# SarodYatawatta/federated-pytorch-test

Hardware: NVIDIA H100
Metric: train_images_per_sec (higher is better)
Workload: dtype tf32

## Files before the change

### federated_pytorch_test_b200/_ext.py

```python
from __future__ import annotations

import importlib.util
import os
import sys
import threading
from typing import Dict, List

_HERE = os.path.dirname(os.path.abspath(__file__))
_CSRC = os.path.join(_HERE, "csrc")
_BUILD = os.path.join(_HERE, "_build")

CUDA_ARCH_FLAGS = ["-gencode", "arch=compute_90a,code=sm_90a"]
NVCC_FLAGS = ["-O3", "-lineinfo", "--use_fast_math", "-std=c++17", "--expt-relaxed-constexpr",
              "-Xptxas", "-v"] + CUDA_ARCH_FLAGS
CXX_FLAGS = ["-O3", "-std=c++17", "-fPIC"]

_SPECS: Dict[str, Dict] = {
    "fedb200_runtime": {"sources": ["batch_loader.cpp"], "cuda": False},
    "fedb200_cuda": {
        "sources": ["bindings.cpp", "flat_kernels.cu", "elementwise_kernels.cu", "norm_kernels.cu", "loss_kernels.cu",
                    "comm_kernels.cu", "gemm_wgmma.cu", "aux_kernels.cu"],
        "cuda": True,
    },
}

_loaded: Dict[str, object] = {}
_lock = threading.Lock()


def _sources(name: str) -> List[str]:
    return [os.path.join(_CSRC, s) for s in _SPECS[name]["sources"] if os.path.exists(os.path.join(_CSRC, s))]


def _so_path(name: str) -> str:
    return os.path.join(_BUILD, name, name + ".so")


def _stale(name: str) -> bool:
    so = _so_path(name)
    if not os.path.exists(so):
        return True
    t = os.path.getmtime(so)
    deps = _sources(name) + [os.path.join(_CSRC, f) for f in os.listdir(_CSRC) if f.endswith((".cuh", ".h", ".hpp"))]
    return any(os.path.getmtime(s) > t for s in deps)
# ... 59 lines not shown
```

### federated_pytorch_test_b200/csrc/bindings.cpp

```cpp
#include <ATen/cuda/CUDAContext.h>
#include <c10/cuda/CUDAGuard.h>
#include <torch/extension.h>

#include <cstdlib>

#include "fedb200.h"

namespace fb = fedb200;
using torch::Tensor;

static cudaStream_t cur_stream() { return at::cuda::getCurrentCUDAStream().stream(); }
static const float* fptr(const Tensor& t) { return t.data_ptr<float>(); }
static float* fptr_mut(Tensor& t) { return t.data_ptr<float>(); }
static const float* opt_ptr(const c10::optional<Tensor>& t) { return (t.has_value() && t->defined()) ? t->data_ptr<float>() : nullptr; }

#define CHECK_F32_CUDA(x) TORCH_CHECK((x).is_cuda() && (x).scalar_type() == torch::kFloat32, #x " must be a CUDA float32 tensor")
#define CHECK_CONTIG(x) TORCH_CHECK((x).is_contiguous(), #x " must be contiguous")

void adam_prox(Tensor x, Tensor g, Tensor m, Tensor v, Tensor step, double lr, double b1, double b2, double eps,
               c10::optional<Tensor> z, c10::optional<Tensor> y, double rho, double l1, double l2,
               c10::optional<Tensor> rho_dev, c10::optional<Tensor> lr_dev, double weight_decay,
               c10::optional<Tensor> norm_dev, double clip) {
  CHECK_F32_CUDA(x); CHECK_CONTIG(x); CHECK_CONTIG(g); CHECK_CONTIG(m); CHECK_CONTIG(v);
  c10::cuda::CUDAGuard guard(x.device());
// ... 183 lines not shown
  fb::col_stats(fptr(y), fptr_mut(stats), (int)(y.numel() / C), C, cur_stream());
}
std::vector<Tensor> bn_elu_fwd(Tensor y, c10::optional<Tensor> stats, Tensor gamma, Tensor beta, c10::optional<Tensor> residual,
                               c10::optional<Tensor> running_mean, c10::optional<Tensor> running_var, double eps,
                               double momentum, bool act, bool self_clean, bool use_running) {
  CHECK_F32_CUDA(y); CHECK_CONTIG(y);
  c10::cuda::CUDAGuard guard(y.device());
  const int C = (int)y.size(-1);
  const int M = (int)(y.numel() / C);
  auto out = torch::empty_like(y);
  float* rm = (running_mean.has_value() && running_mean->defined()) ? running_mean->data_ptr<float>() : nullptr;
  float* rv = (running_var.has_value() && running_var->defined()) ? running_var->data_ptr<float>() : nullptr;
  if (use_running) {
    TORCH_CHECK(rm != nullptr && rv != nullptr, "bn_elu_fwd: use_running needs running_mean and running_var");
    fb::bn_elu_fwd(fptr(y), nullptr, fptr(gamma), fptr(beta), opt_ptr(residual), fptr_mut(out), rm, rv, nullptr, nullptr, M, C,
                   (float)eps, 0.f, act ? 1 : 0, 0, cur_stream(), 1);
    return {out, Tensor(), Tensor()};
  }
  TORCH_CHECK(stats.has_value() && stats->defined(), "bn_elu_fwd: stats required");
  auto sm = torch::empty({C}, y.options()), si = torch::empty({C}, y.options());
  TORCH_CHECK(stats->numel() >= 2 * C + (self_clean ? 1 : 0), "stats buffer too small");
  fb::bn_elu_fwd(fptr(y), stats->data_ptr<float>(), fptr(gamma), fptr(beta), opt_ptr(residual), fptr_mut(out), rm, rv, fptr_mut(sm),
                 fptr_mut(si), M, C, (float)eps, (float)momentum, act ? 1 : 0, self_clean ? 1 : 0, cur_stream());
  return {out, sm, si};
}
std::vector<Tensor> bn_elu_bwd(Tensor dout, c10::optional<Tensor> out, Tensor y, Tensor mean, Tensor invstd, Tensor gamma,
                               c10::optional<Tensor> beta, c10::optional<Tensor> dgamma, c10::optional<Tensor> dbeta,
                               bool want_dres, bool act, c10::optional<Tensor> sums_buf) {
  CHECK_F32_CUDA(dout); CHECK_CONTIG(dout); CHECK_CONTIG(y);
  c10::cuda::CUDAGuard guard(y.device());
  const int C = (int)y.size(-1);
  const int M = (int)(y.numel() / C);
  const float* outp = nullptr;
  if (out.has_value() && out->defined()) { CHECK_CONTIG((*out)); outp = out->data_ptr<float>(); }
  const float* betap = opt_ptr(beta);
  const bool persistent = sums_buf.has_value() && sums_buf->defined();
  if (persistent) TORCH_CHECK(sums_buf->numel() == 2 * C + 1 && sums_buf->is_contiguous(), "bn_elu_bwd: sums buffer must be [2C + 1]");
  auto sums = persistent ? *sums_buf : torch::empty({2 * C + 1}, y.options());
  auto dy = torch::empty_like(y);
  Tensor dres;
  if (want_dres) dres = torch::empty_like(y);
  float* dg = (dgamma.has_value() && dgamma->defined()) ? dgamma->data_ptr<float>() : nullptr;
  float* db = (dbeta.has_value() && dbeta->defined()) ? dbeta->data_ptr<float>() : nullptr;
  fb::bn_elu_bwd_reduce(fptr(dout), outp, fptr(y), fptr(mean), fptr(invstd), fptr(gamma), betap, fptr_mut(sums), M, C,
                        act ? 1 : 0, persistent ? 1 : 0, cur_stream());
  fb::bn_elu_bwd_apply(fptr(dout), outp, fptr(y), fptr(mean), fptr(invstd), fptr(gamma), betap, fptr_mut(sums), fptr_mut(dy),
// ... 851 lines not shown
  m.def("scaffold_corr_blocks", &scaffold_corr_blocks);
  m.def("scaffold_corr", &scaffold_corr);
  m.def("bump_step", &bump_step);
  m.def("l1_l2", &l1_l2);
  m.def("make_pair", &make_pair);
  m.def("welford", &welford);
  m.def("penalty_value", &penalty_value);
  m.def("penalty_grad", &penalty_grad);
  m.def("multi_dot", &multi_dot);
  m.def("lbfgs_two_loop", &lbfgs_two_loop);
  m.def("normalize_u8", &normalize_u8);
  m.def("augment_normalize_u8", &augment_normalize_u8, py::arg("u8"), py::arg("rows"), py::arg("key"), py::arg("counter"),
        py::arg("mean"), py::arg("std"), py::arg("to_nchw"));
  m.def("mix_normalize_u8", &mix_normalize_u8, py::arg("u8"), py::arg("rows"), py::arg("augment"), py::arg("key"),
        py::arg("counter"), py::arg("mean"), py::arg("std"), py::arg("to_nchw"), py::arg("cutmix"), py::arg("lam_f"),
        py::arg("mlam_f"), py::arg("y0"), py::arg("y1"), py::arg("x0"), py::arg("x1"), py::arg("lam_eff"));
  m.def("col_stats", &col_stats);
  m.def("head_fwd", &head_fwd);
  m.def("head_bwd", &head_bwd);
  m.def("bn_elu_fwd", &bn_elu_fwd, py::arg("y"), py::arg("stats"), py::arg("gamma"), py::arg("beta"), py::arg("residual"),
        py::arg("running_mean"), py::arg("running_var"), py::arg("eps"), py::arg("momentum"), py::arg("act"),
        py::arg("self_clean"), py::arg("use_running") = false);
  m.def("bn_elu_bwd", &bn_elu_bwd);
  m.def("gn_elu_fwd", &gn_elu_fwd, py::arg("y"), py::arg("gamma"), py::arg("beta"), py::arg("residual"), py::arg("groups"),
        py::arg("eps"), py::arg("act"));
  m.def("gn_elu_bwd", &gn_elu_bwd, py::arg("dout"), py::arg("out"), py::arg("y"), py::arg("mean"), py::arg("rstd"),
        py::arg("gamma"), py::arg("beta"), py::arg("groups"), py::arg("want_dres"), py::arg("act"), py::arg("want_affine"));
  m.def("avgpool_nhwc", &avgpool_nhwc);
  m.def("avgpool_nhwc_bwd", &avgpool_nhwc_bwd);
  m.def("weight_flip", &weight_flip);
  m.def("convT_pack", &convT_pack);
  m.def("linear_tf32", &linear_tf32);
  m.def("conv_supported", &conv_supported);
  m.def("conv_orientation", &conv_orientation);
  m.def("conv_window_reuse", &conv_window_reuse, py::arg("H_out"), py::arg("W_out"), py::arg("C_in"), py::arg("C_out"), py::arg("kh"),
        py::arg("stride") = 1, py::arg("dil") = 1);
  m.def("conv2d_nhwc", &conv2d_nhwc, py::arg("x"), py::arg("w"), py::arg("stats"), py::arg("stride"), py::arg("pad"), py::arg("dil"),
        py::arg("orient") = -1);
  m.def("conv2d_nhwc_sized", &conv2d_nhwc_sized);
  m.def("conv2d_nhwc_bias_act", &conv2d_nhwc_bias_act);
  m.def("conv2d_nhwc_bn_eval", &conv2d_nhwc_bn_eval);
  m.def("conv2d_nhwc_shuffle", &conv2d_nhwc_shuffle);
  m.def("conv_shuffle_supported", &conv_shuffle_supported);
  m.def("conv2d_nhwc_multidil", &conv2d_nhwc_multidil);
  m.def("conv_multidil_supported", &conv_multidil_supported);
  m.def("conv_wgrad", &conv_wgrad);
// ... 37 lines not shown
```

### federated_pytorch_test_b200/csrc/fedb200.h

```cpp
#pragma once
#include <cuda_runtime.h>
#include <stdint.h>

namespace fedb200 {

void count_launch(int n = 1);
long long launch_count();

bool pdl_enabled();
#ifdef __CUDACC__
__device__ __forceinline__ void pdl_wait() { asm volatile("griddepcontrol.wait;" ::: "memory"); }
__device__ __forceinline__ void pdl_launch_dependents() { asm volatile("griddepcontrol.launch_dependents;" ::: "memory"); }
__device__ __forceinline__ void pdl_prologue() {
  pdl_launch_dependents();
  pdl_wait();
}
template <typename... KArgs, typename... Args>
inline cudaError_t launch_pdl(void (*kernel)(KArgs...), dim3 grid, dim3 block, size_t smem, cudaStream_t stream,
                              Args&&... args) {
  cudaLaunchConfig_t cfg{};
  cfg.gridDim = grid;
  cfg.blockDim = block;
  cfg.dynamicSmemBytes = smem;
  cfg.stream = stream;
// ... 14 lines not shown
int pick_conv_orientation(int NB, int H_out, int W_out, int C_out, int stride);
bool conv_window_reuse(int H_out, int W_out, int C_in, int C_out, int kh, int stride, int dil);
void conv2d_nhwc_tf32(const float* x, const float* w, float* y, float* stats, int NB, int H, int W, int C_in, int C_out,
                      int kh, int kw, int stride, int pad, int dil, int H_out, int W_out, cudaStream_t stream,
                      int orient = CONV_ORIENT_AUTO);
void conv2d_nhwc_bias_act_tf32(const float* x, const float* w, const float* bias, int act, float* y, int NB, int H, int W,
                               int C_in, int C_out, int kh, int kw, int stride, int pad, int dil, int H_out, int W_out,
                               cudaStream_t stream);
void conv2d_nhwc_bn_eval_tf32(const float* x, const float* w, const float* gamma, const float* beta, const float* mean,
                              const float* var, float eps, const float* residual, int act, float* y, int NB, int H, int W,
                              int C_in, int C_out, int kh, int kw, int stride, int pad, int dil, int H_out, int W_out,
                              cudaStream_t stream);

bool conv_shuffle_supported(int H_out, int W_out, int C_in, int Ci_out);
void conv2d_nhwc_shuffle_tf32(const float* x, const float* w, float* out, int NB, int H, int W, int C_in, int C4, int kh, int kw,
                              int pad, int H_out, int W_out, cudaStream_t stream);
bool conv_multidil_supported(int H_out, int W_out, int C_in, int stride, int branches);
void conv2d_nhwc_multidil_tf32(const float* x, const float* w, const float* bias, int act, float* y, int NB, int H, int W, int C_in,
                               int C_out, int branches, int kh, int kw, int stride, const int* dils, const int* pads, int H_out,
                               int W_out, cudaStream_t stream);
bool conv_wgrad_supported(int C_x, int C_out, int stride, int W_out, int H_out);
void conv_wgrad_tf32(const float* x, const float* dy, float* dw, int NB, int H, int W, int C_x, int C_w, int C_out, int kh,
                     int kw, int stride, int pad, int dil, int H_out, int W_out, cudaStream_t stream);


void adam_prox(float* x, const float* g, float* m, float* v, const int* step_dev, int n, float lr, float b1, float b2,
               float eps, const float* z, const float* y, float rho, float l1, float l2, cudaStream_t s,
               const float* rho_dev = nullptr, const float* lr_dev = nullptr, float weight_decay = 0.f,
               const float* norm_dev = nullptr, float clip = 0.f);
void sgd_prox(float* x, const float* g, float* buf, int n, float lr, float momentum, bool nesterov, float weight_decay,
              const float* z, const float* y, float rho, float l1, float l2, cudaStream_t s, const float* rho_dev,
              const float* lr_dev = nullptr, const float* norm_dev = nullptr, float clip = 0.f);
constexpr int kGradNormHeader = 4;
int grad_norm_blocks(int n);
void grad_norm(const float* g, int n, float* ws, unsigned int* ticket, float clip, cudaStream_t s);
void bump_step(int* step_dev, cudaStream_t s);
void l1_l2(const float* g, int n, float* out2, cudaStream_t s);
void make_pair(const float* g, const float* gprev, const float* d, float t, float trust, float* y, float* sv, int n,
               float* out3, cudaStream_t s);
void welford(const float* g, float* mean, float* m2, int n, float inv_n, float* out1, cudaStream_t s);
void penalty_value(const float* x, const float* z, const float* y, float rho, float l1, float l2, int n, float* out1,
                   cudaStream_t s);
void penalty_grad(float* g, const float* x, const float* z, const float* y, float rho, float l1, float l2, int n,
                  cudaStream_t s);
void multi_dot(const float* const* a, const float* const* b, int npairs, int n, float* out, cudaStream_t s);
constexpr int kTwoLoopMaxHist = 32;
// ... 241 lines not shown
```

### federated_pytorch_test_b200/csrc/gemm_wgmma.cu

```cuda
#include "fedb200.h"
#include "igemm_wgmma.cuh"
#include "wgrad_wgmma.cuh"

#include <algorithm>
#include <cstdlib>
#include <mutex>
#include <stdexcept>
#include <string>

namespace fedb200 {

typedef CUresult (*EncodeTiledFn)(CUtensorMap*, CUtensorMapDataType, cuuint32_t, void*, const cuuint64_t*,
                                  const cuuint64_t*, const cuuint32_t*, const cuuint32_t*, CUtensorMapInterleave,
                                  CUtensorMapSwizzle, CUtensorMapL2promotion, CUtensorMapFloatOOBfill);

static EncodeTiledFn encode_fn() {
  static EncodeTiledFn fn = nullptr;
  static std::once_flag once;
  std::call_once(once, [] {
    void* p = nullptr;
    cudaDriverEntryPointQueryResult q;
    cudaError_t e = cudaGetDriverEntryPoint("cuTensorMapEncodeTiled", &p, cudaEnableDefault, &q);
    if (e != cudaSuccess || q != cudaDriverEntryPointSuccess || p == nullptr)
      throw std::runtime_error("fedb200: cuTensorMapEncodeTiled unavailable (no CUDA driver?)");
// ... 402 lines not shown
    p.cw = cw;
    p.num_k_blocks = (kh_all * kw + IG_BLOCK_K / cw - 1) / (IG_BLOCK_K / cw);
  }
  p.taps_w = kw; p.b_cols_per_tap = C_in; p.is_conv = 1;
  p.HW_out = H_out * W_out; p.W_out = W_out;
  p.stride = stride; p.pad = 0; p.dil = 1;
  p.out = y; p.ldo = C_out; p.bias = bias; p.act = act; p.stats = nullptr;
  p.k_splits = 1; p.kb_per_split = p.num_k_blocks;
  p.ms_kh = kh;
  for (int b = 0; b < branches; ++b) {
    if (dils[b] < 1 || dils[b] > 255 || pads[b] < 0 || pads[b] > 255) throw std::runtime_error("fedb200: multi-dilation: dilation / padding out of range");
    p.ms_dil |= (unsigned long long)(dils[b]) << (8 * b);
    p.ms_pad |= (unsigned long long)(pads[b]) << (8 * b);
  }
  dispatch(bn, ta, tb, p, stream);
}

bool conv_wgrad_supported(int C_x, int C_out, int stride, int W_out, int H_out) {
  if ((C_x & 3) || (C_out & 3)) return false;
  if (stride < 1 || stride > 8) return false;
  return W_out > 0 && H_out > 0;
}

template <int BN>
static void launch_wgrad(const float* x, const float* dy, const WgradParams& p, int grid, cudaStream_t stream) {
  constexpr int smem = 2 * (WG_A_BYTES + BN * WG_BK * 4);
  auto kernel = wgrad_wgmma_kernel<BN>;
  static bool configured = false;
  if (!configured) {
    cudaError_t e = cudaFuncSetAttribute(kernel, cudaFuncAttributeMaxDynamicSharedMemorySize, smem);
    if (e != cudaSuccess) throw std::runtime_error(std::string("fedb200: cudaFuncSetAttribute(wgrad): ") + cudaGetErrorString(e));
    configured = true;
  }
  cudaError_t e = launch_pdl(kernel, dim3(grid), dim3(WG_THREADS), size_t(smem), stream, x, dy, p);
  if (e != cudaSuccess) throw std::runtime_error(std::string("fedb200: wgrad launch: ") + cudaGetErrorString(e));
  count_launch();
}

void conv_wgrad_tf32(const float* x, const float* dy, float* dw, int NB, int H, int W, int C_x, int C_w, int C_out, int kh,
                     int kw, int stride, int pad, int dil, int H_out, int W_out, cudaStream_t stream) {
  if (!conv_wgrad_supported(C_x, C_out, stride, W_out, H_out))
    throw std::runtime_error("fedb200: wgrad geometry not supported by the wgmma path");
  WgradParams p{};
  p.H = H; p.W = W; p.Cx = C_x; p.Cw = C_w; p.Co = C_out;
  p.kw = kw; p.stride = stride; p.pad = pad; p.dil = dil; p.H_out = H_out; p.W_out = W_out;
  p.J = kh * kw * C_w;
  p.P = NB * H_out * W_out;
  p.dw = dw;
  const int bn = C_out <= 32 ? 32 : (C_out <= 64 ? 64 : 128);
  p.j_tiles = (p.J + WG_BM - 1) / WG_BM;
  p.co_tiles = (C_out + bn - 1) / bn;
  const int kb_total = (p.P + WG_BK - 1) / WG_BK;
  const int base = p.j_tiles * p.co_tiles;
  int splits = std::max(1, 2 * num_sms() / base);
  splits = std::min(splits, std::max(1, kb_total / 8));
  splits = std::max(1, std::min(splits, kb_total));
  p.kb_per_split = (kb_total + splits - 1) / splits;
  splits = (kb_total + p.kb_per_split - 1) / p.kb_per_split;
  const int grid = base * splits;
  switch (bn) {
    case 32: launch_wgrad<32>(x, dy, p, grid, stream); break;
    case 64: launch_wgrad<64>(x, dy, p, grid, stream); break;
    default: launch_wgrad<128>(x, dy, p, grid, stream); break;
  }
}

}
```

### federated_pytorch_test_b200/csrc/wgrad_wgmma.cuh

```cuda
#pragma once
#include "sm90.cuh"

namespace fedb200 {

constexpr int WG_THREADS = 256;
constexpr int WG_BM = 128;
constexpr int WG_BK = 32;
constexpr int WG_A_BYTES = WG_BM * WG_BK * 4;

struct WgradParams {
  int H, W, Cx, Cw, Co, kw, stride, pad, dil, H_out, W_out;
  int J;
  int P;
  int kb_per_split;
  int j_tiles, co_tiles;
  float* dw;
};

__device__ __forceinline__ uint32_t wg_core_offset(int row, int k) {
  return uint32_t((row >> 3) * 1024 + (k >> 2) * 128 + (row & 7) * 16 + (k & 3) * 4);
}
__device__ __forceinline__ float to_tf32(float v) {
  uint32_t r;
  asm("cvt.rna.tf32.f32 %0, %1;" : "=r"(r) : "f"(v));
  return __uint_as_float(r);
}

template <int BN>
__global__ void __launch_bounds__(WG_THREADS, 1)
wgrad_wgmma_kernel(const float* __restrict__ x, const float* __restrict__ dy, const WgradParams p) {
  constexpr int B_BYTES = BN * WG_BK * 4;
  constexpr int BUF_BYTES = WG_A_BYTES + B_BYTES;
  constexpr int A_PER = WG_BM * WG_BK / WG_THREADS;
  constexpr int B_GROUPS = WG_THREADS / BN;
  constexpr int B_PER = WG_BK / B_GROUPS;
  constexpr int NACC = BN / 2;
  extern __shared__ __align__(1024) uint8_t smem[];

  const int tid = threadIdx.x;
  const int g = tid >> 7, warp = (tid >> 5) & 3, lane = tid & 31;
  int unit = blockIdx.x;
  const int jt = unit % p.j_tiles;
  unit /= p.j_tiles;
  const int ct = unit % p.co_tiles;
  const int split = unit / p.co_tiles;
  const int j0 = jt * WG_BM, co0 = ct * BN;
  const int kb_begin = split * p.kb_per_split;
  const int kb_total = (p.P + WG_BK - 1) / WG_BK;
  const int nkb = min(p.kb_per_split, kb_total - kb_begin);
  const int HWo = p.H_out * p.W_out;

  const int a_row = tid & (WG_BM - 1), a_pg = tid >> 7;
  const int j = j0 + a_row;
// ... 82 lines not shown
```

### federated_pytorch_test_b200/ops/cuda_ops.py

```python
from __future__ import annotations

from typing import List, Optional, Sequence, Tuple

import torch
import torch.nn as nn
import torch.nn.functional as F

from .. import _ext
from . import conv_math

_EXT = None


def ext():
    global _EXT
    if _EXT is None:
        _EXT = _ext.load("fedb200_cuda", required=True)
    return _EXT


def launch_count() -> int:
    return int(ext().launch_count())


# ... 330 lines not shown
    return bool(ext().conv_wgrad_supported(xn.shape[3], dy.shape[3], stride, dy.shape[2], dy.shape[1]))


def conv_wgrad(xn: torch.Tensor, dy: torch.Tensor, kh: int, kw: int, cw: int, stride: int, pad: int, dil: int,
               weight: Optional[torch.Tensor] = None) -> Optional[torch.Tensor]:
    Co = dy.shape[3]
    dyc = dy if dy.is_contiguous() else dy.contiguous()
    buf = _grad_buffer_krsc(weight, (Co, kh, kw, cw))
    if buf is not None:
        ext().conv_wgrad(xn, dyc, buf, stride, pad, dil)
        return None
    dwk = torch.zeros(Co, kh, kw, cw, dtype=torch.float32, device=xn.device)
    ext().conv_wgrad(xn, dyc, dwk, stride, pad, dil)
    return dwk.permute(0, 3, 1, 2)


class _ConvBnAct(torch.autograd.Function):

    @staticmethod
    def forward(ctx, x, weight, gamma, beta, residual, running_mean, running_var, stride, pad, eps, momentum, act):
        e = ext()
        xn = _nhwc(x)
        wk = _krsc(weight)
        if xn.shape[3] == 3:
            xn = F.pad(xn, (0, 1))
            wk = F.pad(wk, (0, 1))
        Co = weight.shape[0]
        stats, self_clean = _stats_buffer(weight, Co)
        y = e.conv2d_nhwc(xn, wk, stats, stride, pad, 1)
        res = _nhwc(residual) if residual is not None else None
        out, mean, invstd = e.bn_elu_fwd(y, stats, gamma, beta, res, running_mean, running_var, eps, momentum, act, self_clean)
        ctx.save_for_backward(xn, wk, y, out, mean, invstd, gamma, beta)
        ctx.cfg = (stride, pad, act, residual is not None, tuple(weight.shape), x.shape[1])
        ctx.w_persistent = _aliases(wk, weight)
        ctx.weight_ref = weight
        return out.permute(0, 3, 1, 2)

    @staticmethod
    def backward(ctx, dout):
        e = ext()
        xn, wk, y, out, mean, invstd, gamma, beta = ctx.saved_tensors
        stride, pad, act, has_res, wshape, cin_logical = ctx.cfg
        need_x, need_w, need_g, need_b, need_r = ctx.needs_input_grad[:5]
        dn = _nhwc(dout)
        dgamma = torch.zeros_like(gamma) if need_g else None
        dbeta = torch.zeros_like(gamma) if need_b else None
        dy, dres = e.bn_elu_bwd(dn, out if (has_res or not act) else None, y, mean, invstd, gamma, beta, dgamma, dbeta,
                                bool(has_res and need_r), act, _bwd_sums_buffer(gamma, gamma.numel()))
        dx, dw = _conv_backward(e, xn, wk, dy, stride, pad, wshape, cin_logical, need_x, need_w, ctx.w_persistent,
                                ctx.weight_ref)
        dr = dres.permute(0, 3, 1, 2) if (has_res and need_r and dres is not None) else None
        return dx, dw, dgamma, dbeta, dr, None, None, None, None, None, None, None
# ... 317 lines not shown
    if tuple(conv.stride) != (1, 1) or tuple(conv.dilation) != (1, 1):
        return False
    kh, kw = conv.kernel_size
    Ho, Wo = x.shape[2] + 2 * conv.padding[0] - kh + 1, x.shape[3] + 2 * conv.padding[1] - kw + 1
    return Ho >= 1 and Wo >= 1 and Ho * Wo <= 64 and conv.in_channels * kh * kw >= 64


def unfold_conv(x: torch.Tensor, conv: nn.Conv2d, act: bool) -> torch.Tensor:
    N, C, H, W = x.shape
    kh, kw = conv.kernel_size
    Ho, Wo = H + 2 * conv.padding[0] - kh + 1, W + 2 * conv.padding[1] - kw + 1
    xp = F.pad(x, (conv.padding[1], conv.padding[1], conv.padding[0], conv.padding[0])) if (conv.padding[0] or conv.padding[1]) else x
    rows = xp.unfold(2, kh, 1).unfold(3, kw, 1).permute(0, 2, 3, 1, 4, 5).reshape(N * Ho * Wo, C * kh * kw)
    out = _LinearAct.apply(rows, conv.weight.reshape(conv.out_channels, C * kh * kw), conv.bias, bool(act))
    return out.view(N, Ho, Wo, conv.out_channels).permute(0, 3, 1, 2)


def conv_act(x: torch.Tensor, conv: nn.Module, act: bool = True) -> torch.Tensor:
    if isinstance(conv, nn.ConvTranspose2d):
        return _ConvTransposeAct.apply(x, conv.weight, conv.bias, bool(act))
    return _ConvAct.apply(x, conv.weight, conv.bias, conv.stride[0], conv.padding[0], conv.dilation[0], bool(act))


def conv_bn_act(x, conv: nn.Conv2d, bn: nn.BatchNorm2d, residual=None, act: bool = True) -> torch.Tensor:
    return _ConvBnAct.apply(x, conv.weight, bn.weight, bn.bias, residual, bn.running_mean, bn.running_var,
                            conv.stride[0], conv.padding[0], bn.eps, bn.momentum, bool(act))


def pool_linear_supported(x, linear, window) -> bool:
    return x.dim() == 4 and x.shape[2] == window and x.shape[3] == window and x.dtype == torch.float32


class _AvgPoolNHWC(torch.autograd.Function):
    @staticmethod
    def forward(ctx, x):
        xn = _nhwc(x)
        ctx.hw = (xn.shape[1], xn.shape[2])
        return ext().avgpool_nhwc(xn)

    @staticmethod
    def backward(ctx, dout):
        dx = ext().avgpool_nhwc_bwd(dout.contiguous(), ctx.hw[0], ctx.hw[1])
        return dx.permute(0, 3, 1, 2)


def _dense_wgrad(dz: torch.Tensor, x: torch.Tensor, wparam) -> Optional[torch.Tensor]:
    e = ext()
# ... 273 lines not shown
```

Baseline: 36640.

## Add dedicated stem conv+BN kernel and small-J wgrad tile path

Adds a dedicated CUDA kernel for the 3-to-64 channel 3x3 stem convolution. It computes the conv with mma.sync TF32 and accumulates BN statistics, with modes to store y, compute stats only, or apply BN+ELU. This avoids padding the input to 4 channels and the general implicit-GEMM path. It also adds a 64-row wgrad tile variant for layers with a tiny reduction dimension such as the stem, cutting wasted tile work. A profiling script is added as well. The no-grad path recomputes the conv twice, and the new code adds maintenance surface.

```diff
diff --git a/baseline/profile_step.py b/baseline/profile_step.py
--- /dev/null
+++ b/baseline/profile_step.py
@@ -0,0 +1,142 @@
+from __future__ import annotations
+
+import argparse
+import collections
+import json
+import os
+import re
+import subprocess
+import sys
+import tempfile
+
+import torch
+
+ROOT = os.path.dirname(os.path.dirname(os.path.abspath(__file__)))
+if ROOT not in sys.path:
+    sys.path.insert(0, ROOT)
+
+STEPS_PER_ROUND = 49
+FIRST_STEP = 12
+
+
+def _power_limit() -> str:
+    try:
+        out = subprocess.run(["nvidia-smi", "--query-gpu=power.limit,clocks.max.sm", "--format=csv,noheader"],
+                             capture_output=True, text=True, timeout=30)
+        return out.stdout.strip().splitlines()[torch.cuda.current_device()] if out.returncode == 0 else "unknown"
+    except (OSError, subprocess.SubprocessError, IndexError):
+        return "unknown"
+
+
+def short_name(name: str) -> str:
+    name = re.sub(r"^void ", "", name)
+    depth = 0
+    for i, ch in enumerate(name):
+        if ch == "<":
+            depth += 1
+        elif ch == ">":
+            depth -= 1
+        elif ch == "(" and depth == 0:
+            return name[:i]
+    return name
+
+
+def stem_kernels(kernels, steps: int) -> dict:
+    out = collections.defaultdict(float)
+    after_stem_conv = False
+    def base(name):
+        return name.split("<")[0].split("::")[-1]
+
+    for i, (name, dur) in enumerate(kernels):
+        b = base(name)
+        if b == "stem_conv_bn_kernel" or b + name[len(name.split("<")[0]):] == "igemm_wgmma_pix_kernel<64, 4, 0>":
+            out["conv (" + name + ")"] += dur
+            after_stem_conv = b != "stem_conv_bn_kernel" or name.endswith("<0>")
+        elif b == "bn_elu_fwd_kernel" and after_stem_conv:
+            out["bn_elu_fwd"] += dur
+            after_stem_conv = False
+        elif b == "wgrad_wgmma_kernel":
+            out["wgrad (" + name + ")"] += dur
+            for want in ("bn_elu_bwd_apply_kernel", "bn_elu_bwd_reduce_kernel"):
+                for j in range(i - 1, -1, -1):
+                    if base(kernels[j][0]) == want:
+                        out[want.replace("_kernel", "")] += kernels[j][1]
+                        break
+    res = {k: v / steps for k, v in out.items()}
+    res["total"] = sum(res.values())
+    return res
+
+
+def main(argv=None) -> dict:
+    ap = argparse.ArgumentParser(description=__doc__.split("\n")[0])
+    ap.add_argument("--steps", type=int, default=20, help="profiled steps (ends before step %d)" % STEPS_PER_ROUND)
+    ap.add_argument("--top", type=int, default=25, help="kernel groups printed")
+    args = ap.parse_args(argv)
+    if not torch.cuda.is_available():
+        raise SystemExit("profile_step.py profiles the GPU step: no CUDA device")
+    if not 1 <= args.steps <= STEPS_PER_ROUND - FIRST_STEP - 1:
+        ap.error("--steps must leave the window inside the first round")
+
+    from torch.profiler import ProfilerActivity, profile
+
+    from federated_pytorch_test_b200.algo.engine import Engine
+    from federated_pytorch_test_b200.algo.strategies import FedAvg
+    from federated_pytorch_test_b200.api import common, federated_multi
+
+    cfg = federated_multi.Config(K=1, use_resnet=True, Nloop=1000, Nadmm=3, Nepoch=1, check_results=False, save_model=False,
+                                 be_verbose=False, biased_input=True, data_on_device=True, graphs=True, fast=True,
+                                 collective="auto", diagnostics="post", max_minibatches=STEPS_PER_ROUND, seed=69,
+                                 optimizer="adam")
+    topo, coll = common.setup_runtime(cfg)
+    task = common.ClassifierTask(cfg, topo, cfg.lambda1, cfg.lambda2)
+    eng = Engine(task, topo, FedAvg(coll, topo), coll, common.engine_config(cfg), log=lambda m: None)
+    dev = topo.device
+    last = FIRST_STEP + args.steps
+    prof = profile(activities=[ProfilerActivity.CUDA])
+
+    def hook(e):
+        n = e.steps_done
+        if n == FIRST_STEP:
+            torch.cuda.synchronize(dev)
+            prof.__enter__()
+        elif n == last:
+            torch.cuda.synchronize(dev)
+            prof.__exit__(None, None, None)
+            e.stop_requested = True
+
+    eng.step_hook = hook
+    eng.run()
+
+    with tempfile.TemporaryDirectory() as tmp:
+        path = os.path.join(tmp, "trace.json")
+        prof.export_chrome_trace(path)
+        with open(path) as f:
+            trace = json.load(f)
+    evs = sorted((e for e in trace["traceEvents"] if e.get("cat") == "kernel"), key=lambda e: e["ts"])
+    kernels = [(short_name(e["name"]), float(e["dur"])) for e in evs]
+    groups = collections.defaultdict(lambda: [0.0, 0])
+    for name, dur in kernels:
+        groups[name][0] += dur
+        groups[name][1] += 1
+    S = args.steps
+    total = sum(d for _, d in kernels) / S
+    table = sorted(((v[0] / S, v[1] / S, k) for k, v in groups.items()), reverse=True)
+    stem = stem_kernels(kernels, S)
+
+    res = {"device": torch.cuda.get_device_name(dev), "power_limit,max_sm_clock": _power_limit(), "steps": S,
+           "kernel_us_per_step": total, "launches_per_step": len(kernels) / S,
+           "kernels": [{"name": k, "us_per_step": t, "launches_per_step": c} for t, c, k in table],
+           "stem_us_per_step": stem}
+    print("device: %s  (power.limit, clocks.max.sm: %s)" % (res["device"], res["power_limit,max_sm_clock"]))
+    print("%d profiled steps: %.1f us of kernel time and %.1f launches per step" % (S, total, len(kernels) / S))
+    for t, c, k in table[:args.top]:
+        print("  %9.1f us  %5.1f x  %s" % (t, c, k[:110]))
+    print("stem, per step:")
+    for k, v in stem.items():
+        print("  %9.1f us  %s" % (v, k))
+    print(json.dumps(res))
+    return res
+
+
+if __name__ == "__main__":
+    main()
diff --git a/federated_pytorch_test_b200/_ext.py b/federated_pytorch_test_b200/_ext.py
--- a/federated_pytorch_test_b200/_ext.py
+++ b/federated_pytorch_test_b200/_ext.py
@@ -19,7 +19,7 @@
     "fedb200_runtime": {"sources": ["batch_loader.cpp"], "cuda": False},
     "fedb200_cuda": {
         "sources": ["bindings.cpp", "flat_kernels.cu", "elementwise_kernels.cu", "norm_kernels.cu", "loss_kernels.cu",
-                    "comm_kernels.cu", "gemm_wgmma.cu", "aux_kernels.cu"],
+                    "comm_kernels.cu", "gemm_wgmma.cu", "aux_kernels.cu", "stem_kernels.cu"],
         "cuda": True,
     },
 }
diff --git a/federated_pytorch_test_b200/csrc/bindings.cpp b/federated_pytorch_test_b200/csrc/bindings.cpp
--- a/federated_pytorch_test_b200/csrc/bindings.cpp
+++ b/federated_pytorch_test_b200/csrc/bindings.cpp
@@ -229,6 +229,42 @@
   TORCH_CHECK(stats->numel() >= 2 * C + (self_clean ? 1 : 0), "stats buffer too small");
   fb::bn_elu_fwd(fptr(y), stats->data_ptr<float>(), fptr(gamma), fptr(beta), opt_ptr(residual), fptr_mut(out), rm, rv, fptr_mut(sm),
                  fptr_mut(si), M, C, (float)eps, (float)momentum, act ? 1 : 0, self_clean ? 1 : 0, cur_stream());
+  return {out, sm, si};
+}
+bool stem_conv_supported(int64_t H, int64_t W, int64_t C_in, int64_t C_out) {
+  return fb::stem_conv_supported((int)H, (int)W, (int)C_in, (int)C_out);
+}
+std::vector<Tensor> stem_conv_bn(Tensor x, Tensor w, Tensor stats, int64_t mode, c10::optional<Tensor> gamma,
+                                 c10::optional<Tensor> beta, c10::optional<Tensor> running_mean, c10::optional<Tensor> running_var,
+                                 double eps, double momentum, bool act, bool self_clean) {
+  CHECK_F32_CUDA(x); CHECK_CONTIG(x); CHECK_F32_CUDA(w); CHECK_CONTIG(w); CHECK_F32_CUDA(stats);
+  TORCH_CHECK(x.dim() == 4 && w.dim() == 4 && x.size(3) == 3 && w.size(0) == 64 && w.size(1) == 3 && w.size(2) == 3 &&
+                  w.size(3) == 3 && fb::stem_conv_supported((int)x.size(1), (int)x.size(2), 3, 64),
+              "stem_conv_bn: x [N,H,32,3] with H % 4 == 0, w [64,3,3,3]");
+  TORCH_CHECK(stats.numel() >= 2 * 64 + 1 && stats.is_contiguous(), "stem_conv_bn: stats buffer too small");
+  TORCH_CHECK(x.size(0) * x.size(1) * x.size(2) * 64 < (int64_t(1) << 31), "stem_conv_bn: batch too large");
+  c10::cuda::CUDAGuard guard(x.device());
+  const int NB = (int)x.size(0), H = (int)x.size(1);
+  if (mode == fb::STEM_STATS_ONLY) {
+    fb::stem_conv_bn(fb::STEM_STATS_ONLY, fptr(x), fptr(w), nullptr, fptr_mut(stats), nullptr, nullptr, nullptr, nullptr, nullptr,
+                     nullptr, NB, H, 0.f, 0.f, 0, 0, cur_stream());
+    return {};
+  }
+  auto out = torch::empty({NB, H, x.size(2), 64}, x.options());
+  if (mode == fb::STEM_STORE_Y) {
+    fb::stem_conv_bn(fb::STEM_STORE_Y, fptr(x), fptr(w), fptr_mut(out), fptr_mut(stats), nullptr, nullptr, nullptr, nullptr,
+                     nullptr, nullptr, NB, H, 0.f, 0.f, 0, 0, cur_stream());
+    return {out};
+  }
+  TORCH_CHECK(mode == fb::STEM_APPLY, "stem_conv_bn: mode must be 0 (STORE_Y), 1 (STATS_ONLY) or 2 (APPLY)");
+  TORCH_CHECK(gamma.has_value() && gamma->defined() && beta.has_value() && beta->defined(), "stem_conv_bn: APPLY needs gamma and beta");
+  CHECK_F32_CUDA((*gamma)); CHECK_F32_CUDA((*beta));
+  float* rm = (running_mean.has_value() && running_mean->defined()) ? running_mean->data_ptr<float>() : nullptr;
+  float* rv = (running_var.has_value() && running_var->defined()) ? running_var->data_ptr<float>() : nullptr;
+  TORCH_CHECK((rm == nullptr) == (rv == nullptr), "stem_conv_bn: running_mean and running_var go together");
+  auto sm = torch::empty({64}, x.options()), si = torch::empty({64}, x.options());
+  fb::stem_conv_bn(fb::STEM_APPLY, fptr(x), fptr(w), fptr_mut(out), fptr_mut(stats), fptr(*gamma), fptr(*beta), rm, rv,
+                   fptr_mut(sm), fptr_mut(si), NB, H, (float)eps, (float)momentum, act ? 1 : 0, self_clean ? 1 : 0, cur_stream());
   return {out, sm, si};
 }
 std::vector<Tensor> bn_elu_bwd(Tensor dout, c10::optional<Tensor> out, Tensor y, Tensor mean, Tensor invstd, Tensor gamma,
@@ -1126,6 +1162,10 @@
         py::arg("running_mean"), py::arg("running_var"), py::arg("eps"), py::arg("momentum"), py::arg("act"),
         py::arg("self_clean"), py::arg("use_running") = false);
   m.def("bn_elu_bwd", &bn_elu_bwd);
+  m.def("stem_conv_supported", &stem_conv_supported);
+  m.def("stem_conv_bn", &stem_conv_bn, py::arg("x"), py::arg("w"), py::arg("stats"), py::arg("mode"), py::arg("gamma") = py::none(),
+        py::arg("beta") = py::none(), py::arg("running_mean") = py::none(), py::arg("running_var") = py::none(),
+        py::arg("eps") = 1e-5, py::arg("momentum") = 0.1, py::arg("act") = true, py::arg("self_clean") = false);
   m.def("gn_elu_fwd", &gn_elu_fwd, py::arg("y"), py::arg("gamma"), py::arg("beta"), py::arg("residual"), py::arg("groups"),
         py::arg("eps"), py::arg("act"));
   m.def("gn_elu_bwd", &gn_elu_bwd, py::arg("dout"), py::arg("out"), py::arg("y"), py::arg("mean"), py::arg("rstd"),
diff --git a/federated_pytorch_test_b200/csrc/fedb200.h b/federated_pytorch_test_b200/csrc/fedb200.h
--- a/federated_pytorch_test_b200/csrc/fedb200.h
+++ b/federated_pytorch_test_b200/csrc/fedb200.h
@@ -60,6 +60,12 @@
 bool conv_wgrad_supported(int C_x, int C_out, int stride, int W_out, int H_out);
 void conv_wgrad_tf32(const float* x, const float* dy, float* dw, int NB, int H, int W, int C_x, int C_w, int C_out, int kh,
                      int kw, int stride, int pad, int dil, int H_out, int W_out, cudaStream_t stream);
+
+enum { STEM_STORE_Y = 0, STEM_STATS_ONLY = 1, STEM_APPLY = 2 };
+bool stem_conv_supported(int H, int W, int C_in, int C_out);
+void stem_conv_bn(int mode, const float* x, const float* w, float* out, float* stats, const float* gamma, const float* beta,
+                  float* running_mean, float* running_var, float* save_mean, float* save_invstd, int NB, int H, float eps,
+                  float momentum, int act, int self_clean, cudaStream_t stream);
 
 
 void adam_prox(float* x, const float* g, float* m, float* v, const int* step_dev, int n, float lr, float b1, float b2,
diff --git a/federated_pytorch_test_b200/csrc/gemm_wgmma.cu b/federated_pytorch_test_b200/csrc/gemm_wgmma.cu
--- a/federated_pytorch_test_b200/csrc/gemm_wgmma.cu
+++ b/federated_pytorch_test_b200/csrc/gemm_wgmma.cu
@@ -448,10 +448,10 @@
   return W_out > 0 && H_out > 0;
 }
 
-template <int BN>
+template <int BN, int BM = WG_BM>
 static void launch_wgrad(const float* x, const float* dy, const WgradParams& p, int grid, cudaStream_t stream) {
-  constexpr int smem = 2 * (WG_A_BYTES + BN * WG_BK * 4);
-  auto kernel = wgrad_wgmma_kernel<BN>;
+  constexpr int smem = 2 * (BM * WG_BK * 4 + BN * WG_BK * 4);
+  auto kernel = wgrad_wgmma_kernel<BN, BM>;
   static bool configured = false;
   if (!configured) {
     cudaError_t e = cudaFuncSetAttribute(kernel, cudaFuncAttributeMaxDynamicSharedMemorySize, smem);
@@ -474,7 +474,8 @@
   p.P = NB * H_out * W_out;
   p.dw = dw;
   const int bn = C_out <= 32 ? 32 : (C_out <= 64 ? 64 : 128);
-  p.j_tiles = (p.J + WG_BM - 1) / WG_BM;
+  const bool small_j = kh * kw * C_x <= WG_BM_SMALL && (reinterpret_cast<uintptr_t>(x) & 15) == 0;
+  p.j_tiles = small_j ? 1 : (p.J + WG_BM - 1) / WG_BM;
   p.co_tiles = (C_out + bn - 1) / bn;
   const int kb_total = (p.P + WG_BK - 1) / WG_BK;
   const int base = p.j_tiles * p.co_tiles;
@@ -484,6 +485,14 @@
   p.kb_per_split = (kb_total + splits - 1) / splits;
   splits = (kb_total + p.kb_per_split - 1) / p.kb_per_split;
   const int grid = base * splits;
+  if (small_j) {
+    switch (bn) {
+      case 32: launch_wgrad<32, WG_BM_SMALL>(x, dy, p, grid, stream); break;
+      case 64: launch_wgrad<64, WG_BM_SMALL>(x, dy, p, grid, stream); break;
+      default: launch_wgrad<128, WG_BM_SMALL>(x, dy, p, grid, stream); break;
+    }
+    return;
+  }
   switch (bn) {
     case 32: launch_wgrad<32>(x, dy, p, grid, stream); break;
     case 64: launch_wgrad<64>(x, dy, p, grid, stream); break;
diff --git a/federated_pytorch_test_b200/csrc/stem_kernels.cu b/federated_pytorch_test_b200/csrc/stem_kernels.cu
--- /dev/null
+++ b/federated_pytorch_test_b200/csrc/stem_kernels.cu
@@ -0,0 +1,276 @@
+#include "fedb200.h"
+
+#include <stdexcept>
+#include <string>
+
+namespace fedb200 {
+
+namespace {
+
+constexpr int STEM_ROWS = 4;
+constexpr int STEM_THREADS = 32 * STEM_ROWS;
+constexpr int STEM_W = 32;
+constexpr int STEM_CI = 3, STEM_CO = 64, STEM_K = 27;
+constexpr int STEM_WIN_W = STEM_W + 2;
+constexpr int STEM_WIN = (STEM_ROWS + 2) * STEM_WIN_W * STEM_CI;
+constexpr int STEM_CTAS_PER_SM = 4;
+
+int stem_sm_count() {
+  static int n = 0;
+  if (n == 0) {
+    int dev = 0;
+    cudaGetDevice(&dev);
+    cudaDeviceGetAttribute(&n, cudaDevAttrMultiProcessorCount, dev);
+    if (n <= 0) n = 132;
+  }
+  return n;
+}
+
+__device__ __forceinline__ float stem_tf32(float v) {
+  uint32_t r;
+  asm("cvt.rn.tf32.f32 %0, %1;" : "=r"(r) : "f"(v));
+  return __uint_as_float(r);
+}
+__device__ __forceinline__ float stem_elu(float v) { return v > 0.f ? v : (__expf(v) - 1.f); }
+
+__device__ __forceinline__ void mma_tf32_16x8x8(float (&d)[4], const float (&a)[4], float b0, float b1) {
+  asm volatile("mma.sync.aligned.m16n8k8.row.col.f32.tf32.tf32.f32 {%0, %1, %2, %3}, {%4, %5, %6, %7}, {%8, %9}, "
+               "{%0, %1, %2, %3};"
+               : "+f"(d[0]), "+f"(d[1]), "+f"(d[2]), "+f"(d[3])
+               : "r"(__float_as_uint(a[0])), "r"(__float_as_uint(a[1])), "r"(__float_as_uint(a[2])), "r"(__float_as_uint(a[3])),
+                 "r"(__float_as_uint(b0)), "r"(__float_as_uint(b1)));
+}
+
+struct StemParams {
+  const float* x;
+  const float* w;
+  float* out;
+  float* stats;
+  const float* gamma;
+  const float* beta;
+  float* running_mean;
+  float* running_var;
+  float* save_mean;
+  float* save_invstd;
+  int H;
+  int bands;
+  float eps, momentum;
+  int act, self_clean;
+};
+
+}
+
+template <int MODE>
+__global__ void __launch_bounds__(STEM_THREADS, STEM_CTAS_PER_SM)
+stem_conv_bn_kernel(const StemParams p) {
+  constexpr bool STORE = MODE != STEM_STATS_ONLY;
+  constexpr int WIN_PER = (STEM_WIN + STEM_THREADS - 1) / STEM_THREADS;
+  __shared__ float xs[2][STEM_WIN];
+  __shared__ __align__(16) float wf[8 * 4 * 32 * 2];
+  __shared__ __align__(16) float stage[STORE ? STEM_ROWS * STEM_W * STEM_CO : 4];
+  __shared__ float red[STEM_ROWS][2 * STEM_CO];
+  __shared__ float bn_sc[STEM_CO], bn_sh[STEM_CO];
+  __shared__ int last_block;
+
+  const int tid = threadIdx.x, warp = tid >> 5, lane = tid & 31;
+  const int g = lane >> 2, t = lane & 3;
+  const int per_img = p.H / STEM_ROWS;
+  const int M = p.bands * STEM_ROWS * STEM_W;
+
+  float pre[WIN_PER];
+  auto fetch = [&](int band) {
+    const int n = band / per_img, h0 = (band - n * per_img) * STEM_ROWS;
+    const float* xn = p.x + size_t(n) * p.H * STEM_W * STEM_CI;
+#pragma unroll
+    for (int u = 0; u < WIN_PER; ++u) {
+      const int i = tid + u * STEM_THREADS;
+      const int r = i / (STEM_WIN_W * STEM_CI), rem = i - r * (STEM_WIN_W * STEM_CI);
+      const int c = rem / STEM_CI, ci = rem - c * STEM_CI;
+      const int h = h0 - 1 + r, w = c - 1;
+      pre[u] = (i < STEM_WIN && h >= 0 && h < p.H && w >= 0 && w < STEM_W) ? __ldg(xn + (h * STEM_W + w) * STEM_CI + ci) : 0.f;
+    }
+  };
+  auto put = [&](int buf) {
+#pragma unroll
+    for (int u = 0; u < WIN_PER; ++u) {
+      const int i = tid + u * STEM_THREADS;
+      if (i < STEM_WIN) xs[buf][i] = stem_tf32(pre[u]);
+    }
+  };
+
+  pdl_prologue();
+  int band = blockIdx.x;
+  fetch(band);
+  for (int i = tid; i < 8 * 4 * 32 * 2; i += STEM_THREADS) {
+    const int e = i & 1, l = (i >> 1) & 31, kk = (i >> 6) & 3, j = i >> 8;
+    const int k = 8 * kk + (l & 3) + 4 * e;
+    wf[i] = k < STEM_K ? stem_tf32(__ldg(p.w + (8 * j + (l >> 2)) * STEM_K + k)) : 0.f;
+  }
+  if constexpr (MODE == STEM_APPLY) {
+    if (tid < STEM_CO) {
+      const float invM = 1.f / float(M);
+      const float mean = p.stats[tid] * invM;
+      float var = fmaf(-mean, mean, p.stats[STEM_CO + tid] * invM);
+      var = var > 0.f ? var : 0.f;
+      const float invstd = rsqrtf(var + p.eps);
+      const float sc = p.gamma[tid] * invstd;
+      bn_sc[tid] = sc;
+      bn_sh[tid] = fmaf(-mean, sc, p.beta[tid]);
+      if (blockIdx.x == 0) {
+        p.save_mean[tid] = mean;
+        p.save_invstd[tid] = invstd;
+        if (p.running_mean != nullptr) {
+          const float unbiased = M > 1 ? var * float(M) / float(M - 1) : var;
+          p.running_mean[tid] = fmaf(p.momentum, mean - p.running_mean[tid], p.running_mean[tid]);
+          p.running_var[tid] = fmaf(p.momentum, unbiased - p.running_var[tid], p.running_var[tid]);
+        }
+      }
+    }
+  }
+  put(0);
+  __syncthreads();
+  if constexpr (MODE == STEM_APPLY) {
+    if (p.self_clean) {
+      unsigned int* counter = reinterpret_cast<unsigned int*>(p.stats + 2 * STEM_CO);
+      if (tid == 0) {
+        __threadfence();
+        last_block = atomicAdd(counter, 1u) == gridDim.x - 1;
+      }
+      __syncthreads();
+      if (last_block) {
+        for (int c = tid; c < 2 * STEM_CO; c += STEM_THREADS) p.stats[c] = 0.f;
+        if (tid == 0) *counter = 0u;
+      }
+    }
+  }
+
+  int koff[4][2];
+#pragma unroll
+  for (int kk = 0; kk < 4; ++kk)
+#pragma unroll
+    for (int e = 0; e < 2; ++e) {
+      const int k = 8 * kk + t + 4 * e, tap = k / STEM_CI, ci = k - tap * STEM_CI;
+      koff[kk][e] = k < STEM_K ? ((tap / 3) * STEM_WIN_W + tap % 3) * STEM_CI + ci : -1;
+    }
+  if constexpr (MODE != STEM_APPLY) {
+    for (int c = lane; c < 2 * STEM_CO; c += 32) red[warp][c] = 0.f;
+    __syncwarp();
+  }
+
+  for (int it = 0; band < p.bands; band += gridDim.x, ++it) {
+    const int buf = it & 1;
+    const int next = band + gridDim.x;
+    const float* xw = xs[buf];
+    float* st = stage + warp * STEM_W * STEM_CO;
+    if constexpr (STORE) __syncwarp();
+#pragma unroll 1
+    for (int mt = 0; mt < 2; ++mt) {
+      float acc[8][4];
+#pragma unroll
+      for (int j = 0; j < 8; ++j)
+#pragma unroll
+        for (int q = 0; q < 4; ++q) acc[j][q] = 0.f;
+      const int p0 = (warp * STEM_WIN_W + 16 * mt + g) * STEM_CI;
+#pragma unroll
+      for (int kk = 0; kk < 4; ++kk) {
+        float a[4];
+#pragma unroll
+        for (int e = 0; e < 2; ++e) {
+          const bool ok = koff[kk][e] >= 0;
+          a[2 * e] = ok ? xw[p0 + koff[kk][e]] : 0.f;
+          a[2 * e + 1] = ok ? xw[p0 + 8 * STEM_CI + koff[kk][e]] : 0.f;
+        }
+#pragma unroll
+        for (int j = 0; j < 8; ++j) {
+          const float2 b = *reinterpret_cast<const float2*>(&wf[((j * 4 + kk) * 32 + lane) * 2]);
+          mma_tf32_16x8x8(acc[j], a, b.x, b.y);
+        }
+      }
+
+#pragma unroll
+      for (int j = 0; j < 8; ++j) {
+        if constexpr (MODE != STEM_APPLY) {
+#pragma unroll
+          for (int e = 0; e < 2; ++e) {
+            const float v0 = acc[j][e], v1 = acc[j][2 + e];
+            float a1 = v0 + v1, a2 = fmaf(v1, v1, v0 * v0);
+#pragma unroll
+            for (int o = 4; o < 32; o <<= 1) {
+              a1 += __shfl_xor_sync(0xffffffffu, a1, o);
+              a2 += __shfl_xor_sync(0xffffffffu, a2, o);
+            }
+            if (g == 0) {
+              red[warp][8 * j + 2 * t + e] += a1;
+              red[warp][STEM_CO + 8 * j + 2 * t + e] += a2;
+            }
+          }
+        }
+        if constexpr (STORE) {
+#pragma unroll
+          for (int hh = 0; hh < 2; ++hh) {
+            const int px = 16 * mt + g + 8 * hh, c = 8 * j + 2 * t;
+            float v0 = acc[j][2 * hh], v1 = acc[j][2 * hh + 1];
+            if constexpr (MODE == STEM_APPLY) {
+              v0 = fmaf(v0, bn_sc[c], bn_sh[c]);
+              v1 = fmaf(v1, bn_sc[c + 1], bn_sh[c + 1]);
+              if (p.act) { v0 = stem_elu(v0); v1 = stem_elu(v1); }
+            }
+            *reinterpret_cast<float2*>(st + px * STEM_CO + (((c >> 2) ^ (px & 15)) << 2) + (c & 3)) = make_float2(v0, v1);
+          }
+        }
+      }
+    }
+    if (next < p.bands) fetch(next);
+    if constexpr (STORE) {
+      __syncwarp();
+      const int n = band / per_img, h0 = (band - n * per_img) * STEM_ROWS;
+      float4* dst = reinterpret_cast<float4*>(p.out + ((size_t(n) * p.H + h0 + warp) * STEM_W) * STEM_CO);
+      const float4* src = reinterpret_cast<const float4*>(st);
+#pragma unroll
+      for (int i = 0; i < STEM_W * STEM_CO / 4 / 32; ++i) {
+        const int idx = 32 * i + lane, px = idx >> 4, q = idx & 15;
+        dst[idx] = src[px * 16 + (q ^ (px & 15))];
+      }
+    }
+    if (next < p.bands) put(buf ^ 1);
+    __syncthreads();
+  }
+
+  if constexpr (MODE != STEM_APPLY) {
+    float a = 0.f;
+#pragma unroll
+    for (int w = 0; w < STEM_ROWS; ++w) a += red[w][tid];
+    atomicAdd(p.stats + tid, a);
+  }
+}
+
+bool stem_conv_supported(int H, int W, int C_in, int C_out) {
+  return W == STEM_W && H > 0 && H % STEM_ROWS == 0 && C_in == STEM_CI && C_out == STEM_CO;
+}
+
+void stem_conv_bn(int mode, const float* x, const float* w, float* out, float* stats, const float* gamma, const float* beta,
+                  float* running_mean, float* running_var, float* save_mean, float* save_invstd, int NB, int H, float eps,
+                  float momentum, int act, int self_clean, cudaStream_t stream) {
+  if (!stem_conv_supported(H, STEM_W, STEM_CI, STEM_CO) || NB <= 0)
+    throw std::runtime_error("fedb200: stem_conv_bn needs [N, H, 32, 3] input with H % 4 == 0 and 64 output channels");
+  if ((mode == STEM_STORE_Y || mode == STEM_APPLY) && (reinterpret_cast<uintptr_t>(out) & 15))
+    throw std::runtime_error("fedb200: stem_conv_bn needs a 16-byte aligned output");
+  if (mode == STEM_APPLY && (gamma == nullptr || beta == nullptr || save_mean == nullptr || save_invstd == nullptr))
+    throw std::runtime_error("fedb200: stem_conv_bn APPLY needs gamma, beta, save_mean and save_invstd");
+  const int bands = NB * (H / STEM_ROWS);
+  StemParams p{x, w, out, stats, gamma, beta, running_mean, running_var, save_mean, save_invstd, H, bands, eps, momentum, act,
+               self_clean};
+  const int per_cta = (bands + STEM_CTAS_PER_SM * stem_sm_count() - 1) / (STEM_CTAS_PER_SM * stem_sm_count());
+  const dim3 grid((bands + per_cta - 1) / per_cta);
+  cudaError_t e;
+  switch (mode) {
+    case STEM_STORE_Y: e = launch_pdl(stem_conv_bn_kernel<STEM_STORE_Y>, grid, dim3(STEM_THREADS), 0, stream, p); break;
+    case STEM_STATS_ONLY: e = launch_pdl(stem_conv_bn_kernel<STEM_STATS_ONLY>, grid, dim3(STEM_THREADS), 0, stream, p); break;
+    case STEM_APPLY: e = launch_pdl(stem_conv_bn_kernel<STEM_APPLY>, grid, dim3(STEM_THREADS), 0, stream, p); break;
+    default: throw std::runtime_error("fedb200: stem_conv_bn: unknown mode");
+  }
+  if (e != cudaSuccess) throw std::runtime_error(std::string("fedb200: stem_conv_bn launch: ") + cudaGetErrorString(e));
+  count_launch();
+}
+
+}
diff --git a/federated_pytorch_test_b200/csrc/wgrad_wgmma.cuh b/federated_pytorch_test_b200/csrc/wgrad_wgmma.cuh
--- a/federated_pytorch_test_b200/csrc/wgrad_wgmma.cuh
+++ b/federated_pytorch_test_b200/csrc/wgrad_wgmma.cuh
@@ -7,6 +7,7 @@
 constexpr int WG_BM = 128;
 constexpr int WG_BK = 32;
 constexpr int WG_A_BYTES = WG_BM * WG_BK * 4;
+constexpr int WG_BM_SMALL = 64;
 
 struct WgradParams {
   int H, W, Cx, Cw, Co, kw, stride, pad, dil, H_out, W_out;
@@ -27,8 +28,142 @@
 }
 
 template <int BN>
+__device__ __forceinline__ void wgrad_small_j(const float* __restrict__ x, const float* __restrict__ dy, const WgradParams& p) {
+  constexpr int A_BYTES = WG_BM_SMALL * WG_BK * 4;
+  constexpr int B_BYTES = BN * WG_BK * 4;
+  constexpr int BUF_BYTES = A_BYTES + B_BYTES;
+  constexpr int QUADS = WG_BM_SMALL / 4;
+  constexpr int A_GROUPS = WG_THREADS / QUADS;
+  constexpr int A_PER = WG_BK / A_GROUPS;
+  constexpr int B_GROUPS = WG_THREADS / BN;
+  constexpr int B_PER = WG_BK / B_GROUPS;
+  constexpr int NACC = BN / 2;
+  static_assert(2 * BUF_BYTES >= WG_THREADS / 2 * NACC * 4, "the cross-warpgroup sum reuses the operand buffers");
+  extern __shared__ __align__(1024) uint8_t smem[];
+
+  const int tid = threadIdx.x;
+  const int g = tid >> 7, warp = (tid >> 5) & 3, lane = tid & 31;
+  int unit = blockIdx.x;
+  const int ct = unit % p.co_tiles;
+  const int split = unit / p.co_tiles;
+  const int co0 = ct * BN;
+  const int kb_begin = split * p.kb_per_split;
+  const int kb_total = (p.P + WG_BK - 1) / WG_BK;
+  const int nkb = min(p.kb_per_split, kb_total - kb_begin);
+  const int HWo = p.H_out * p.W_out;
+  const int taps = p.J / p.Cw;
+  const int Jx = taps * p.Cx;
+
+  const int a_q = (tid >> 2) & (QUADS - 1), a_pg = (tid & 3) | ((tid >> 6) << 2);
+  const int j4 = 4 * a_q;
+  const bool j_ok = j4 < Jx;
+  const int tap = j_ok ? j4 / p.Cx : 0;
+  const int ci = j_ok ? j4 - tap * p.Cx : 0;
+  const int dh = (tap / p.kw) * p.dil - p.pad, dwo = (tap % p.kw) * p.dil - p.pad;
+  const int b_row = tid % BN, b_pg = tid / BN;
+  const int co = co0 + b_row;
+  const bool co_ok = co < p.Co;
+
+  float4 ra[A_PER];
+  float rb[B_PER];
+  auto gather = [&](int kb) {
+    const int pbase = (kb_begin + kb) * WG_BK;
+#pragma unroll
+    for (int q = 0; q < A_PER; ++q) {
+      const int pix = pbase + a_pg + A_GROUPS * q;
+      float4 v = make_float4(0.f, 0.f, 0.f, 0.f);
+      if (j_ok && pix < p.P) {
+        const int n = pix / HWo, rem = pix - n * HWo;
+        const int ho = rem / p.W_out, wo = rem - ho * p.W_out;
+        const int h = ho * p.stride + dh, w = wo * p.stride + dwo;
+        if (h >= 0 && h < p.H && w >= 0 && w < p.W)
+          v = __ldg(reinterpret_cast<const float4*>(x + ((size_t(n) * p.H + h) * p.W + w) * p.Cx + ci));
+      }
+      ra[q] = v;
+    }
+#pragma unroll
+    for (int q = 0; q < B_PER; ++q) {
+      const int pix = pbase + b_pg + B_GROUPS * q;
+      rb[q] = (co_ok && pix < p.P) ? __ldg(dy + size_t(pix) * p.Co + co) : 0.f;
+    }
+  };
+  auto scatter = [&](int buf) {
+    uint8_t* a = smem + buf * BUF_BYTES;
+    uint8_t* b = a + A_BYTES;
+#pragma unroll
+    for (int q = 0; q < A_PER; ++q) {
+      const int k = a_pg + A_GROUPS * q;
+      const float v[4] = {ra[q].x, ra[q].y, ra[q].z, ra[q].w};
+#pragma unroll
+      for (int c = 0; c < 4; ++c) *reinterpret_cast<float*>(a + wg_core_offset(j4 + c, k)) = to_tf32(v[c]);
+    }
+#pragma unroll
+    for (int q = 0; q < B_PER; ++q) *reinterpret_cast<float*>(b + wg_core_offset(b_row, b_pg + B_GROUPS * q)) = to_tf32(rb[q]);
+    fence_proxy_async();
+  };
+
+  pdl_launch_dependents();
+  pdl_wait();
+  float acc[NACC];
+#pragma unroll
+  for (int i = 0; i < NACC; ++i) acc[i] = 0.f;
+  const uint32_t base = smem_u32(smem);
+  if (nkb > 0) {
+    gather(0);
+    scatter(0);
+    __syncthreads();
+  }
+  for (int kb = 0; kb < nkb; ++kb) {
+    const int buf = kb & 1;
+    if (kb + 1 < nkb) gather(kb + 1);
+    const uint32_t a_addr = base + uint32_t(buf * BUF_BYTES);
+    const uint32_t b_addr = a_addr + uint32_t(A_BYTES);
+    wgmma_fence();
+    wgmma_fence_acc(acc);
+#pragma unroll
+    for (int kk = 0; kk < WG_BK / 16; ++kk) {
+      const uint32_t k = uint32_t(2 * g + kk);
+      wgmma_tf32<BN>(acc, make_kmajor_interleave_desc(a_addr + 256u * k, 128, 1024),
+                     make_kmajor_interleave_desc(b_addr + 256u * k, 128, 1024), 1u);
+    }
+    wgmma_commit();
+    if (kb + 1 < nkb) scatter(buf ^ 1);
+    wgmma_wait<0>();
+    wgmma_fence_acc(acc);
+    __syncthreads();
+  }
+
+  float* red = reinterpret_cast<float*>(smem);
+  const int t128 = tid & 127;
+  if (g == 1) {
+#pragma unroll
+    for (int i = 0; i < NACC; ++i) red[i * 128 + t128] = acc[i];
+  }
+  __syncthreads();
+  if (g == 1 || nkb <= 0) return;
+#pragma unroll
+  for (int i = 0; i < NACC; ++i) acc[i] += red[i * 128 + t128];
+  const int r_a = 16 * warp + (lane >> 2);
+#pragma unroll
+  for (int i = 0; i < NACC / 4; ++i) {
+#pragma unroll
+    for (int e = 0; e < 4; ++e) {
+      const int jj = r_a + 8 * (e >> 1);
+      const int cc = co0 + 8 * i + 2 * (lane & 3) + (e & 1);
+      const int t_ = jj / p.Cx, c_ = jj - t_ * p.Cx;
+      if (jj < Jx && c_ < p.Cw && cc < p.Co) atomicAdd(p.dw + size_t(cc) * p.J + t_ * p.Cw + c_, acc[4 * i + e]);
+    }
+  }
+}
+
+template <int BN, int BM = WG_BM>
 __global__ void __launch_bounds__(WG_THREADS, 1)
 wgrad_wgmma_kernel(const float* __restrict__ x, const float* __restrict__ dy, const WgradParams p) {
+  static_assert(BM == WG_BM || BM == WG_BM_SMALL, "128- or 64-row tiles");
+  if constexpr (BM == WG_BM_SMALL) {
+    wgrad_small_j<BN>(x, dy, p);
+    return;
+  }
   constexpr int B_BYTES = BN * WG_BK * 4;
   constexpr int BUF_BYTES = WG_A_BYTES + B_BYTES;
   constexpr int A_PER = WG_BM * WG_BK / WG_THREADS;
diff --git a/federated_pytorch_test_b200/ops/cuda_ops.py b/federated_pytorch_test_b200/ops/cuda_ops.py
--- a/federated_pytorch_test_b200/ops/cuda_ops.py
+++ b/federated_pytorch_test_b200/ops/cuda_ops.py
@@ -376,12 +376,19 @@
         e = ext()
         xn = _nhwc(x)
         wk = _krsc(weight)
-        if xn.shape[3] == 3:
-            xn = F.pad(xn, (0, 1))
-            wk = F.pad(wk, (0, 1))
         Co = weight.shape[0]
         stats, self_clean = _stats_buffer(weight, Co)
-        y = e.conv2d_nhwc(xn, wk, stats, stride, pad, 1)
+        if _stem_supported(x, weight, stride, pad, residual):
+            y = e.stem_conv_bn(xn, wk, stats, STEM_STORE_Y)[0]
+            if ctx.needs_input_grad[0] or ctx.needs_input_grad[1]:
+                xn = F.pad(xn, (0, 1))
+            if ctx.needs_input_grad[0]:
+                wk = F.pad(wk, (0, 1))
+        else:
+            if xn.shape[3] == 3:
+                xn = F.pad(xn, (0, 1))
+                wk = F.pad(wk, (0, 1))
+            y = e.conv2d_nhwc(xn, wk, stats, stride, pad, 1)
         res = _nhwc(residual) if residual is not None else None
         out, mean, invstd = e.bn_elu_fwd(y, stats, gamma, beta, res, running_mean, running_var, eps, momentum, act, self_clean)
         ctx.save_for_backward(xn, wk, y, out, mean, invstd, gamma, beta)
@@ -745,7 +752,29 @@
     return _ConvAct.apply(x, conv.weight, conv.bias, conv.stride[0], conv.padding[0], conv.dilation[0], bool(act))
 
 
+STEM_STORE_Y, STEM_STATS_ONLY, STEM_APPLY = 0, 1, 2
+
+
+def _stem_supported(x: torch.Tensor, weight: torch.Tensor, stride: int, pad: int, residual) -> bool:
+    return (residual is None and x.dim() == 4 and tuple(weight.shape) == (64, 3, 3, 3) and stride == 1 and pad == 1
+            and bool(ext().stem_conv_supported(x.shape[2], x.shape[3], 3, 64)))
+
+
+def _stem_bn_act(x: torch.Tensor, conv: nn.Conv2d, bn: nn.BatchNorm2d, act: bool) -> torch.Tensor:
+    e = ext()
+    xn = _nhwc(x)
+    wk = _krsc(conv.weight)
+    stats, self_clean = _stats_buffer(conv.weight, 64)
+    e.stem_conv_bn(xn, wk, stats, STEM_STATS_ONLY)
+    out = e.stem_conv_bn(xn, wk, stats, STEM_APPLY, bn.weight, bn.bias, bn.running_mean, bn.running_var, bn.eps, bn.momentum,
+                         bool(act), self_clean)[0]
+    return out.permute(0, 3, 1, 2)
+
+
 def conv_bn_act(x, conv: nn.Conv2d, bn: nn.BatchNorm2d, residual=None, act: bool = True) -> torch.Tensor:
+    if _stem_supported(x, conv.weight, conv.stride[0], conv.padding[0], residual) and not (
+            torch.is_grad_enabled() and any(t is not None and t.requires_grad for t in (x, conv.weight, bn.weight, bn.bias))):
+        return _stem_bn_act(x, conv, bn, act)
     return _ConvBnAct.apply(x, conv.weight, bn.weight, bn.bias, residual, bn.running_mean, bn.running_var,
                             conv.stride[0], conv.padding[0], bn.eps, bn.momentum, bool(act))
 
```

Result: faster. 38050, median of 6 (+3.8%).
